# mschauer/ZigZagBoomerang.jl

Hardware: AMD Instinct MI355X
Metric: reflection events/sec, d=16384 local ZigZag (spdmp), ensemble of independent chains (higher is better)
Workload: dtype f64

## Files before the change

### include/pdmp_debug.h

```cpp
#ifndef PDMP_DEBUG_H
#define PDMP_DEBUG_H

#include <stddef.h>

#include "pdmp_mi355.h"

#ifdef __cplusplus
extern "C" {
#endif

#define PDMP_DEBUG_KERNEL_AUTO 0
#define PDMP_DEBUG_KERNEL_SEQ 1
#define PDMP_DEBUG_KERNEL_SPEC4 2
#define PDMP_DEBUG_KERNEL_SPEC8 3
#define PDMP_DEBUG_KERNEL_EXACTP 4
pdmp_status pdmp_debug_set_kernel(pdmp_ensemble* ens, int kernel);
pdmp_status pdmp_debug_set_spec_g2(pdmp_ensemble* ens, int on);
pdmp_status pdmp_debug_set_phase_profile(pdmp_ensemble* ens, int on);
pdmp_status pdmp_debug_phase_profile(pdmp_ensemble* ens, double* out16, int* kind);
pdmp_status pdmp_debug_set_track_groups(pdmp_ensemble* ens, int which);
pdmp_status pdmp_debug_set_helper_wave(pdmp_ensemble* ens, int mode);
pdmp_status pdmp_debug_set_track_lines(pdmp_ensemble* ens, int mode);
pdmp_status pdmp_debug_buffer_addresses(pdmp_ensemble* ens, uint64_t* out8);
pdmp_status pdmp_debug_placement(pdmp_ensemble* ens, char* buf, size_t nbuf);
pdmp_status pdmp_debug_set_placement(pdmp_ensemble* ens, int tune, int place, const char* rec, const char* kp, const char* ev);
pdmp_status pdmp_debug_move_buffer(pdmp_ensemble* ens, int which);
pdmp_status pdmp_debug_set_helper_steering(pdmp_ensemble* ens, double gain, int target, double ahead);
pdmp_status pdmp_debug_set_launch_count_limit(pdmp_ensemble* ens, uint32_t n);
pdmp_status pdmp_debug_set_consumer_overlap(pdmp_ensemble* ens, int mode);
pdmp_status pdmp_debug_host_drain_probe(pdmp_ensemble* ens, int64_t bytes, double* gbps);
pdmp_status pdmp_debug_last_kernel(pdmp_ensemble* ens, char* out, int64_t cap);
pdmp_status pdmp_debug_set_logistic_rows(pdmp_ensemble* ens, int row_width);
pdmp_status pdmp_debug_set_proposal_dump(pdmp_ensemble* ens, int64_t n);

pdmp_status pdmp_debug_math_probe(int device, uint64_t seed, int64_t n, double* out);

#define PDMP_MATH_U01 0
#define PDMP_MATH_LOG 1
#define PDMP_MATH_EXP 2
#define PDMP_MATH_SINCOS 3
#define PDMP_MATH_SINCOS2PI 4
#define PDMP_MATH_RANDN 5
#define PDMP_MATH_RANDN2 6
#define PDMP_MATH_RANDINT 7
// ... 41 lines not shown
```

### zigzagboomerang.jl_amd/_lib.py

```python
import ctypes as C
import os

import numpy as np

from . import build as _build

PDMP_OK = 0
ABI_VERSION = 3
ERR_NAMES = {0: "PDMP_OK", 1: "PDMP_ERR_INVALID", 2: "PDMP_ERR_NO_DEVICE", 3: "PDMP_ERR_HIP",
             4: "PDMP_ERR_UNSUPPORTED", 5: "PDMP_ERR_NOMEM"}

PDMP_ERR_INVALID, PDMP_ERR_NO_DEVICE, PDMP_ERR_HIP, PDMP_ERR_UNSUPPORTED, PDMP_ERR_NOMEM = 1, 2, 3, 4, 5
SAMPLER_ZIGZAG_LOCAL, SAMPLER_ZIGZAG_ALL, SAMPLER_BPS, SAMPLER_STICKY_ZIGZAG = 0, 1, 2, 3
CHAIN_OK, CHAIN_BOUND_VIOLATED, CHAIN_STALLED, CHAIN_TRACE_FULL, CHAIN_PAUSED = 0, 1, 2, 3, 4


def needs_rerun(status):
    st = np.asarray(status)
    return bool(np.any((st == CHAIN_TRACE_FULL) | (st == CHAIN_PAUSED)))
RUN_REFERENCE_TAIL, RUN_STOP_BEFORE = 0, 1

EVENT_DTYPE = np.dtype([("t", "<f8"), ("i", "<i8"), ("x", "<f8"), ("theta", "<f8")])
COUNTERS_DTYPE = np.dtype([("t_last", "<f8"), ("num", "<u8"), ("nacc", "<u8"), ("nrefresh", "<u8"),
                           ("ntrace", "<u8"), ("nevents", "<u8"), ("ndraw_main", "<u8"),
                           ("ndraw_global", "<u8"), ("status", "<u4"), ("reserved", "<u4")])
assert EVENT_DTYPE.itemsize == 32 and COUNTERS_DTYPE.itemsize == 72

EXPORTED_SYMBOLS = [
    "pdmp_last_error", "pdmp_abi_version", "pdmp_device_count", "pdmp_ensemble_create",
    "pdmp_ensemble_destroy", "pdmp_ensemble_set_flow_zigzag", "pdmp_ensemble_set_target_gaussian_csc",
    "pdmp_ensemble_set_state", "pdmp_ensemble_set_state_synthetic", "pdmp_ensemble_run", "pdmp_ensemble_run_partitioned", "pdmp_ensemble_sync",
    "pdmp_ensemble_last_run_ms", "pdmp_ensemble_counters", "pdmp_ensemble_totals", "pdmp_ensemble_trace_copy",
    "pdmp_ensemble_trace_reset", "pdmp_ensemble_final_state", "pdmp_ensemble_batch_means",
    "pdmp_ensemble_trace_dev", "pdmp_ensemble_counters_dev", 
    "pdmp_ensemble_set_flow_bps", "pdmp_ensemble_set_state_bps", "pdmp_ensemble_bps_trace_copy",
    "pdmp_ensemble_bps_final_state", "pdmp_ensemble_set_sticky", "pdmp_ensemble_set_adaptscale", "pdmp_ensemble_final_sigma", "pdmp_ensemble_set_flow_boomerang", "pdmp_ensemble_set_local_bound", "pdmp_ensemble_set_target_logistic", "pdmp_ensemble_set_flow_factboomerang",
    "pdmp_ensemble_set_mass_cholesky", "pdmp_ensemble_set_bps_options", "pdmp_ensemble_set_bps_moments", "pdmp_ensemble_bps_moments",
    "pdmp_ensemble_set_bps_sticky", "pdmp_ensemble_bps_trace_free_copy", "pdmp_ensemble_bps_final_sticky",
    "pdmp_ensemble_ess_begin", "pdmp_ensemble_ess_batch", "pdmp_ensemble_ess_end", "pdmp_ensemble_set_gradient_tracking",
    "pdmp_ensemble_path_integrals", "pdmp_ensemble_set_path_integrals", "pdmp_ensemble_set_neighbourhood", "pdmp_ensemble_info",
    "pdmp_ensemble_consume_begin", "pdmp_ensemble_consume", "pdmp_ensemble_consume_async", "pdmp_ensemble_last_consume_ms", "pdmp_ensemble_consume_mean", "pdmp_ensemble_consume_inclusion", "pdmp_ensemble_consume_discretized", "pdmp_ensemble_consume_cummean", "pdmp_ensemble_consume_cummean_copy", "pdmp_ensemble_subtrace_copy", "pdmp_1d_run",
    "pdmp_comm_unique_id", "pdmp_comm_init", "pdmp_comm_destroy", "pdmp_comm_info", "pdmp_comm_barrier", "pdmp_comm_allreduce",
    "pdmp_ensemble_gather_traces", "pdmp_ensemble_reduce_moments", "pdmp_comm_gathered_copy",
    "pdmp_ensemble_gather_bps_traces", "pdmp_comm_gathered_bps_copy", "pdmp_ensemble_bps_trace_dev",
]
DEBUG_SYMBOLS = ["pdmp_debug_set_kernel", "pdmp_debug_set_spec_g2", "pdmp_debug_set_phase_profile", "pdmp_debug_phase_profile",
                 "pdmp_debug_set_proposal_dump", "pdmp_debug_set_track_groups", "pdmp_debug_set_helper_wave", "pdmp_debug_set_track_lines", "pdmp_debug_buffer_addresses", "pdmp_debug_placement", "pdmp_debug_set_placement", "pdmp_debug_move_buffer", "pdmp_debug_set_helper_steering", "pdmp_debug_set_launch_count_limit", "pdmp_debug_host_drain_probe", "pdmp_debug_set_consumer_overlap", "pdmp_debug_last_kernel", "pdmp_debug_set_logistic_rows", "pdmp_debug_math_probe", "pdmp_debug_math_eval", "pdmp_debug_write_probe", "pdmp_debug_sector_probe",
                 "pdmp_debug_sticky_eval"]
DEBUG_KERNELS = {"auto": 0, "seq": 1, "spec4": 2, "spec8": 3, "exactp": 4}


class PdmpConfig(C.Structure):
    _fields_ = [("struct_size", C.c_uint32), ("device", C.c_int32), ("sampler", C.c_int32), ("adapt", C.c_int32),
                ("factor", C.c_double), ("nchains", C.c_int64), ("d", C.c_int64), ("trace_capacity", C.c_int64)]


class PdmpError(RuntimeError):
    def __init__(self, code, msg):
        super().__init__(f"{ERR_NAMES.get(code, code)}: {msg}")
        self.code = code


_lib = None
_loaded_path = None


def loaded_path():
    return _loaded_path


# ... 82 lines not shown
    L.pdmp_ensemble_set_flow_bps.argtypes = [vp, vp, vp, vp, vp, f64, f64]
    L.pdmp_ensemble_set_flow_boomerang.argtypes = [vp, vp, vp, vp, vp, vp, f64, f64]
    L.pdmp_ensemble_set_state_bps.argtypes = [vp, f64, vp, vp, f64, vp]
    L.pdmp_ensemble_ess_begin.argtypes = [vp, f64]
    L.pdmp_ensemble_ess_batch.argtypes = [vp, f64]
    L.pdmp_ensemble_ess_end.argtypes = [vp, vp, vp, vp, vp, C.POINTER(i64), C.POINTER(f64), C.POINTER(f64)]
    L.pdmp_ensemble_set_mass_cholesky.argtypes = [vp, vp, vp, vp]
    L.pdmp_ensemble_set_bps_options.argtypes = [vp, C.c_int, C.c_int]
    L.pdmp_ensemble_set_bps_moments.argtypes = [vp, C.c_int]
    L.pdmp_ensemble_bps_moments.argtypes = [vp, f64, i64, i64, vp, vp]
    L.pdmp_ensemble_set_bps_sticky.argtypes = [vp, vp, C.c_int]
    L.pdmp_ensemble_bps_trace_free_copy.argtypes = [vp, i64, i64, i64, vp]
    L.pdmp_ensemble_bps_final_sticky.argtypes = [vp, i64, i64, vp, vp]
    L.pdmp_debug_sticky_eval.argtypes = [C.c_int, C.c_int, i64, vp, vp, vp, vp]
    L.pdmp_ensemble_bps_trace_copy.argtypes = [vp, i64, i64, i64, vp, vp, vp]
    L.pdmp_ensemble_bps_final_state.argtypes = [vp, i64, i64, vp, vp, vp, vp]
    L.pdmp_debug_set_kernel.argtypes = [vp, C.c_int]
    L.pdmp_debug_set_spec_g2.argtypes = [vp, C.c_int]
    L.pdmp_debug_set_phase_profile.argtypes = [vp, C.c_int]
    L.pdmp_debug_phase_profile.argtypes = [vp, vp, C.POINTER(C.c_int)]
    L.pdmp_debug_set_proposal_dump.argtypes = [vp, i64]
    L.pdmp_debug_set_track_groups.argtypes = [vp, C.c_int]
    L.pdmp_debug_set_helper_wave.argtypes = [vp, C.c_int]
    L.pdmp_debug_set_track_lines.argtypes = [vp, C.c_int]
    L.pdmp_debug_buffer_addresses.argtypes = [vp, C.POINTER(C.c_uint64)]
    L.pdmp_debug_move_buffer.argtypes = [vp, C.c_int]
    L.pdmp_debug_placement.argtypes = [vp, C.c_char_p, C.c_size_t]
    L.pdmp_debug_set_placement.argtypes = [vp, C.c_int, C.c_int, C.c_char_p, C.c_char_p, C.c_char_p]
    L.pdmp_debug_set_launch_count_limit.argtypes = [vp, C.c_uint32]
    L.pdmp_debug_set_helper_steering.argtypes = [vp, C.c_double, C.c_int, C.c_double]
    L.pdmp_debug_last_kernel.argtypes = [vp, C.c_char_p, i64]
    L.pdmp_debug_set_logistic_rows.argtypes = [vp, C.c_int]
    for name in EXPORTED_SYMBOLS + DEBUG_SYMBOLS:
        fn = getattr(L, name)
        if name not in ("pdmp_last_error", "pdmp_abi_version", "pdmp_device_count", "pdmp_ensemble_destroy", "pdmp_comm_destroy"):
            fn.restype = C.c_int
    _lib = L
    _loaded_path = path
    return L


class Config1d(C.Structure):
    _fields_ = [("struct_size", C.c_uint32), ("device", C.c_int32), ("flow", C.c_int32), ("adapt", C.c_int32), ("factor", C.c_double),
                ("nchains", C.c_int64), ("trace_capacity", C.c_int64), ("mu", C.c_double), ("sigma2", C.c_double), ("noise", C.c_double),
                ("b_sigma", C.c_double), ("b_mu", C.c_double), ("b_lambda", C.c_double)]

# ... 41 lines not shown
```

### zigzagboomerang.jl_amd/csrc/pdmp_capi.hip

```cpp
#include <hip/hip_runtime.h>

#include <chrono>

#include <algorithm>
#include <cmath>
#include <cstdarg>
#include <cstdio>
#include <cstdlib>
#include <cstring>
#include <string>
#include <unordered_map>
#include <vector>

#include "../../include/pdmp_detmath.h"
#include "../../include/pdmp_debug.h"
#include "pdmp_engine.hpp"

namespace {

thread_local std::string g_err;
thread_local std::string g_deferred_err;

pdmp_status fail(pdmp_status st, const char* fmt, ...) {
    char buf[512];
// ... 81 lines not shown
    DevBuf<uint64_t> d_blob;
    DevBuf<uint32_t> d_tix;
    size_t n_templates = 0;
    uint32_t common_tix = 0;

    DevBuf<uint32_t> d_colptr, d_rowval, d_sptr, d_sidx, d_qptr;
    DevBuf<uint8_t> d_pos, d_selfpos;
    DevBuf<double> d_bval, d_tval, d_gmu_b, d_gmu_t, d_c, d_c2, d_sigma;
    DevBuf<pdmp::CoordConst> d_cc;
    DevBuf<pdmp::ZzRec> d_rec;
    DevBuf<double> d_keys, d_c_chain, d_jprev, d_sum;
    int dbg_kernel = 0;
    int dbg_lg_rows = -1;
    int dbg_spec_g2 = 0;
    int dbg_phase = 0;
    double dbg_phase_out[16] = {0};
    int dbg_phase_valid = 0;
    int64_t dbg_dump = 0;
    int dbg_track_groups = 0;
    double dbg_hw_steer[3] = {0, 0, 0};
    uint32_t dbg_count_limit = 0;
    int dbg_cons_overlap = -1;
    int n_cu = 0;
    int dbg_helper_wave = -1;
    bool track_requested = false, track = false, track_two_sums = false;
    bool track_lg = false;
    DevBuf<double> d_trk;
    bool exactp = false;
    bool track_pairs = false;
    DevBuf<double> d_kp;
    bool track_lines = false, canon_stale = false;
    pdmp::PlaceConfig place_cfg;
    int place_tune = 1;
    std::string tune_log;
    int dbg_track_lines = -1;
    DevBuf<pdmp::TrLine> d_tl_lines;
    DevBuf<pdmp::TrCold> d_tl_cold;
    bool has_g8 = false, g8_same = false;
    int g8_gw = 8;
    DevBuf<uint64_t> d_g8_line;
    DevBuf<double> d_g8_member, d_g8_gamt;
    bool track_generic = false;
    DevBuf<double> d_gam8;
    DevBuf<uint16_t> d_nb16;
    const char* last_kernel = "";
    int32_t lattice_n = 0;
// ... 416 lines not shown
        return hipSuccess;
    };
    switch (which) {
        case 0: HIP_TRY(move_buf(e->d_rec)); break;
        case 1: HIP_TRY(move_buf(e->d_kp)); break;
        case 2: HIP_TRY(move_buf(e->d_ev)); break;
        case 3: HIP_TRY(move_buf(e->d_hdr)); break;
        case 4: HIP_TRY(move_buf(e->d_cc)); break;
        case 5: HIP_TRY(move_buf(e->d_keys)); break;
        case 6: HIP_TRY(move_buf(e->b_ev_x)); break;
        case 7: HIP_TRY(move_buf(e->b_ev_th)); break;
        case 8: HIP_TRY(move_buf(e->b_x)); break;
        case 9: HIP_TRY(move_buf(e->b_th)); break;
        case 10: HIP_TRY(move_buf(e->b_ev_t)); break;
        default: return fail(PDMP_ERR_INVALID, "move buffer: 0 records, 1 pairs, 2 trace, 3 headers, 4 constants, 5 keys; BPS: 6 / 7 event x / theta, 8 / 9 x / theta, 10 event t");
    }
    return PDMP_OK;
}
pdmp_status pdmp_debug_set_helper_wave(pdmp_ensemble* e, int mode) {
    if (!e || mode < -1 || mode > 1) return fail(PDMP_ERR_INVALID, "helper wave: -1 (by occupancy), 0 (never), 1 (always)");
    e->dbg_helper_wave = mode;
    return PDMP_OK;
}
pdmp_status pdmp_debug_set_consumer_overlap(pdmp_ensemble* e, int mode) {
    if (!e || mode < -1 || mode > 1) return fail(PDMP_ERR_INVALID, "consumer overlap: -1 (by width), 0 (between slices), 1 (beside the next slice)");
    e->dbg_cons_overlap = mode;
    return PDMP_OK;
}
pdmp_status pdmp_debug_set_launch_count_limit(pdmp_ensemble* e, uint32_t n) {
    if (!e) return fail(PDMP_ERR_INVALID, "null argument");
    e->dbg_count_limit = n;
    return PDMP_OK;
}
pdmp_status pdmp_debug_set_helper_steering(pdmp_ensemble* e, double gain, int target, double ahead) {
    if (!e || !(gain > 0.0 && gain <= 4096.0) || target < 1 || target > 64 || !(ahead >= 0.0))
        return fail(PDMP_ERR_INVALID, "helper steering: 0 < gain <= 4096 (<= 1 for the two-wave form), 1 <= target <= 64, ahead >= 0");
    e->dbg_hw_steer[0] = gain;
    e->dbg_hw_steer[1] = (double)target;
    e->dbg_hw_steer[2] = ahead;
    return PDMP_OK;
}
pdmp_status pdmp_debug_set_logistic_rows(pdmp_ensemble* e, int w) {
    if (!e || (w != -1 && w != 0 && w != 16 && w != 32)) return fail(PDMP_ERR_INVALID, "row width: -1 (default), 0 (one chain per wavefront), 16 or 32");
#ifndef PDMP_EXTRA_KERNELS
    if (w > 0) return fail(PDMP_ERR_UNSUPPORTED, "zz_logistic_rows_kernel is not part of this library: it lives in the parity build (build.py --variant parity, -DPDMP_EXTRA_KERNELS)");
#endif
// ... 911 lines not shown
    if (general_path(e)) return P;
    if (e->track || e->exactp) {
        P.lattice_n = e->lattice_n;
        P.lattice_magic = e->lattice_n ? (uint32_t)(((uint64_t)1 << 32) / (uint64_t)e->lattice_n + 1) : 0u;
    }
    if (!e->track) return P;
    P.track_two_sums = e->track_two_sums ? 1 : 0;
    if (!e->track_pairs) return P;
    P.typ_extra = e->typ_extra;
    P.hw_gain = e->dbg_hw_steer[0];
    P.hw_target = (uint32_t)e->dbg_hw_steer[1];
    P.hw_ahead = e->dbg_hw_steer[2];
    if (e->track_lines) {
        P.tl_lines = e->d_tl_lines.p;
        P.tl_cold = e->d_tl_cold.p;
        return P;
    }
    P.keys = e->d_kp.p;
    P.track_mean = e->track_mean;
    if (e->track_mean == 2) P.tb.gmu_t = nullptr;
    P.n_cu = e->n_cu;
    P.helper_wave = (e->dbg_helper_wave == 1 || (e->dbg_helper_wave == -1 && e->cfg.nchains <= (int64_t)HELPER_WAVE_MAX_CHAINS_PER_CU * (e->n_cu > 0 ? e->n_cu : 256))) ? 1 : 0;
    if (pdmp::zz_trackp_big(e->cfg.d)) P.helper_wave = 0;
    return P;
}

static pdmp::ZzGeneralParams general_params(const pdmp_ensemble* e) {
    pdmp::ZzGeneralParams Q{};
    Q.local_bound = e->local_bound ? 1 : 0;
    Q.masked = e->has_g1mask ? 1 : 0;
    Q.sticky = e->cfg.sampler == PDMP_SAMPLER_STICKY_ZIGZAG ? 1 : 0;
    Q.qtval = e->d_qtval.p;
    Q.renew_chain = e->local_bound ? e->d_thf.p : nullptr;
    Q.sig_chain = e->adaptscale ? e->d_sig_chain.p : nullptr;
    Q.adaptscale = e->adaptscale ? 1 : 0;
    Q.pos16 = e->d_pos16.p;
    Q.qbval = e->d_qbval.p;
    Q.member = reinterpret_cast<const uint4*>(e->d_member.p);
    Q.selfpos16 = e->d_selfpos16.p;
    Q.mmax_pad = (e->mmax_all + 63u) & ~63u;
    Q.target_kind = e->target_kind;
    Q.A_colptr = e->lg_Acp.p;
    Q.A_rowval = e->lg_Arv.p;
    Q.A_nzval = e->lg_Anz.p;
    Q.At_colptr = e->lg_Atcp.p;
    Q.At_rowval = e->lg_Atrv.p;
// ... 184 lines not shown

static pdmp::BpsRunParams bps_run_params(const pdmp_ensemble* e, double T, int flags);
static pdmp::BpsMomParams bps_moments_params(const pdmp_ensemble* e);
static pdmp::BpsStickyParams bps_sticky_params(const pdmp_ensemble* e);

pdmp_status pdmp_ensemble_run(pdmp_ensemble* e, double T, int flags, void* stream) {
    pdmp_status st = ensemble_run_impl(e, T, flags, stream);
    if (st == PDMP_OK && e->cfg.sampler != PDMP_SAMPLER_BPS) e->run_T = T;
    if (st == PDMP_OK && e->deferred_k >= 0) st = launch_deferred_consumer(e);
    return st;
}

static pdmp_status ensemble_run_impl(pdmp_ensemble* e, double T, int flags, void* stream) {
    if (!e) return fail(PDMP_ERR_INVALID, "null argument");
    if (!e->has_state) return fail(PDMP_ERR_INVALID, "set_state must be called before run");
    if (flags != PDMP_RUN_REFERENCE_TAIL && flags != PDMP_RUN_STOP_BEFORE) return fail(PDMP_ERR_INVALID, "bad flags");
    HIP_TRY(hipSetDevice(e->cfg.device));
    e->ran = true;
    hipStream_t s = stream ? (hipStream_t)stream : e->stream;
    const int64_t n = e->cfg.nchains;
    const bool bps = e->cfg.sampler == PDMP_SAMPLER_BPS;
    pdmp_status st;
    if (!bps) e->dbg_phase_valid = 0;
    if (!bps && general_path(e) && e->lg_nemax >= 1024 && !e->d_hot.p && (st = e->d_hot.alloc((size_t)n * (size_t)e->cfg.d * 4)) != PDMP_OK) return st;
    const pdmp::BpsRunParams B = bps_run_params(e, T, flags);
    pdmp::ZzRunParams P = run_params(e, T, flags);
    const pdmp::ZzGeneralParams Q = general_params(e);
    const pdmp::ZzLogisticTables LT = logistic_tables(e);
    KernelFamily fam;
    if ((st = select_family(e, P, Q, LT, &fam)) != PDMP_OK) return st;
    const FamilyInfo& F = FAMILY[fam];
    DevBuf<double> dbgbuf, phbuf;
    const int64_t dbg_cap = bps ? 0 : e->dbg_dump;
    if (dbg_cap > 0) {
        if ((st = dbgbuf.alloc((size_t)dbg_cap * 16)) != PDMP_OK) return st;
        HIP_TRY(hipMemsetAsync(dbgbuf.p, 0, (size_t)dbg_cap * 16 * sizeof(double), s));
        P.dbg = dbgbuf.p;
        P.dbg_cap = dbg_cap;
    }
    HIP_TRY(hipEventRecord(e->ev0, s));
    const bool profiled = e->dbg_phase != 0 && F.phase_kind != 0;
    if (profiled) {
        if ((st = phbuf.alloc(16)) != PDMP_OK) return st;
        HIP_TRY(hipMemsetAsync(phbuf.p, 0, 16 * sizeof(double), s));
        P.dbg = phbuf.p;
        P.dbg_cap = 0;
    }
    int rc = 0;
    switch (fam) {
    case FAM_BPS:
        if (e->bps_sticky) {
            e->last_kernel = "bps_sticky_run_kernel";
            rc = pdmp::launch_bps_sticky_run(B, bps_sticky_params(e), n, s);
        } else {
            e->last_kernel = "bps_run_kernel";
            rc = pdmp::launch_bps_run(B, n, e->bps_diag, s, bps_moments_params(e));
        }
        break;
    case FAM_GENERAL: e->last_kernel = "zz_general_run_kernel"; rc = pdmp::launch_zz_general_run(P, Q, n, s); break;
    case FAM_LOGISTIC_LDS: e->last_kernel = "zz_logistic_lds_kernel"; rc = pdmp::launch_zz_logistic_lds(P, Q, LT, e->keep_integrals, n, s); break;
    case FAM_TRACKL: e->last_kernel = "zz_local_trackl_kernel"; e->canon_stale = true; rc = pdmp::launch_zz_local_trackl(P, n, s); break;
    case FAM_TRACKP: rc = pdmp::launch_zz_local_trackp(P, n, s, &e->last_kernel); break;
    case FAM_TRACK_GROUPS: e->last_kernel = "zz_local_track_kernel"; rc = pdmp::launch_zz_local_track(P, n, s); break;
    case FAM_STICKY_SPEC: e->last_kernel = "zz_sticky_spec_kernel"; rc = pdmp::launch_zz_sticky_spec(P, n, s); break;
    case FAM_STICKY_RUN: e->last_kernel = "zz_sticky_run_kernel"; rc = pdmp::launch_zz_sticky_run(P, n, s); break;
    case FAM_SPEC: rc = pdmp::launch_zz_local_spec(P, n, s, &e->last_kernel); break;
    case FAM_ONE_EVENT: e->last_kernel = "zz_local_run_kernel"; rc = pdmp::launch_zz_local_run(P, n, s); break;
#ifdef PDMP_EXTRA_KERNELS
    case FAM_LOGISTIC_ROWS: e->last_kernel = "zz_logistic_rows_kernel"; rc = pdmp::launch_zz_logistic_rows(P, Q, LT, e->keep_integrals, logistic_rows_width(e), n, s); break;
    case FAM_EXACTP: e->last_kernel = "zz_local_exactp_kernel"; rc = pdmp::launch_zz_local_exactp(P, n, s); break;
#else
    case FAM_LOGISTIC_ROWS: case FAM_EXACTP: return fail(PDMP_ERR_UNSUPPORTED, "kernel family %d is not part of this library", (int)fam);
#endif
    }
    if (rc != 0 && F.hip_rc) return fail(PDMP_ERR_HIP, "%s launch failed: %s", F.launcher, hipGetErrorString((hipError_t)rc));
    if (rc != 0) return fail(PDMP_ERR_HIP, "%s launch failed (%d)", F.launcher, rc);
    HIP_TRY(hipEventRecord(e->ev1, s));
    e->timed = true;
    if (profiled) {
        HIP_TRY(device_sync(e));
        HIP_TRY(hipMemcpy(e->dbg_phase_out, phbuf.p, sizeof e->dbg_phase_out, hipMemcpyDeviceToHost));
        e->dbg_phase_valid = F.phase_kind;
    }
    if (dbg_cap > 0 && (fam == FAM_ONE_EVENT || fam == FAM_STICKY_RUN)) {
        HIP_TRY(device_sync(e));
        std::vector<double> hd((size_t)dbg_cap * 16);
        HIP_TRY(hipMemcpy(hd.data(), dbgbuf.p, hd.size() * sizeof(double), hipMemcpyDeviceToHost));
        for (int64_t r = 0; r < dbg_cap; ++r) {
            const double* D = hd.data() + r * 16;
            fprintf(stderr, "DBG %3lld tp=%.6f i=%g acc=%g k=%g m=%g self=%g l=%.6g lb=%.6g u=%.6f key=%.6f t=%.6f L=%.6f g=%.6g a_i=%.6g x0=%.6g cj=%.6g\n",
                    (long long)r, D[0], D[1], D[2], D[3], D[4], D[5], D[6], D[7], D[8], D[9], D[10], D[11], D[12], D[13], D[14], D[15]);
        }
    }
    return PDMP_OK;
}

pdmp_status pdmp_ensemble_sync(pdmp_ensemble* e) {
    if (!e) return fail(PDMP_ERR_INVALID, "null argument");
    HIP_TRY(hipSetDevice(e->cfg.device));
    HIP_TRY(device_sync(e));
    return PDMP_OK;
}

pdmp_status pdmp_ensemble_last_run_ms(pdmp_ensemble* e, float* ms) {
    if (!e || !ms) return fail(PDMP_ERR_INVALID, "null argument");
// ... 1226 lines not shown
```

### zigzagboomerang.jl_amd/csrc/pdmp_engine.hpp

```cpp
#pragma once
#include <cstdint>
#include <string>
#include <vector>

#include "../../include/pdmp_mi355.h"
#ifdef PDMP_EXTRA_KERNELS
#include "../../include/pdmp_debug.h"
#endif

namespace pdmp {

struct alignas(64) ZzRec {
    double x;
    double th;
    double t;
    double I;
    double t_old;
    double a, b;
    uint64_t acc;
};
static_assert(sizeof(ZzRec) == 64, "record must be one 64-byte sector");

struct alignas(128) TrRec {
    double x, th, tx, I;
// ... 98 lines not shown
    uint32_t blob_w, blob_w_pad, blob_sw, blob_pw, blob_kmax;
    uint32_t common_tix;
    int64_t d;
    int64_t dk;
    int64_t trace_cap;
    uint32_t nblk;
    uint32_t nblk_pad;
    double T;
    double factor;
    double lambda_ref;
    int32_t flags;
    int32_t adapt;
    int32_t has_refresh;
    int32_t move_all;
    int32_t force_spec4;
    int32_t track_two_sums;
    int32_t track_mean;
    uint32_t count_limit;
    uint32_t typ_extra;
    double hw_gain, hw_ahead;
    uint32_t hw_target;
    int32_t n_cu;
    int32_t helper_wave;
    void* tl_lines;
    void* tl_cold;
    int32_t lattice_n;
    uint32_t lattice_magic;
    const uint64_t* __restrict__ g8_line;
    const double* __restrict__ g8_member;
    const double* __restrict__ g8_gamt;
    int32_t g8_gw;
    const double* __restrict__ kappa;
    double* thf;
    int32_t reversible, strong_upperbounds;
};

struct ZzInitParams {
    ZzTables tb;
    ZzRec* rec;
    double* keys;
    DevChain* hdr;
    double* c_chain;
    const double* x0;
    const double* th0;
    const uint64_t* seeds;
    uint64_t seed0;
// ... 256 lines not shown
```

### zigzagboomerang.jl_amd/csrc/pdmp_trackp.hip

```cpp
#include <hip/hip_runtime.h>

#include <cstdint>

#include "../../include/pdmp_detmath.h"
#include "pdmp_device.hpp"
#include "pdmp_engine.hpp"

namespace pdmp {

namespace {

__device__ __forceinline__ uint32_t w_grp8_min_u32(uint32_t v) {
    uint32_t o = (uint32_t)__builtin_amdgcn_mov_dpp((int)v, 0xB1, 0xf, 0xf, true);
    v = (o < v) ? o : v;
    o = (uint32_t)__builtin_amdgcn_mov_dpp((int)v, 0x4E, 0xf, 0xf, true);
    v = (o < v) ? o : v;
    o = (uint32_t)__builtin_amdgcn_mov_dpp((int)v, 0x141, 0xf, 0xf, true);
    return (o < v) ? o : v;
}
__device__ __forceinline__ uint32_t p_enc(double key, double tb, uint32_t pos) {
    double dlt = key - tb;
    dlt = (dlt > 0.0) ? dlt : 0.0;
    const uint32_t b = __float_as_uint((float)dlt);
    return (((b >= 8u) ? b - 8u : 0u) & ~7u) | pos;
// ... 221 lines not shown
        uint32_t e = P_INFBITS;
        if (b < nblk) {
            const double2* p = kp + (size_t)b * 8;
            double mk = p[0].x;
            uint32_t mi = 0;
#pragma unroll
            for (int q = 1; q < 8; ++q) {
                const double v = p[q].x;
                if (v < mk) {
                    mk = v;
                    mi = q;
                }
            }
            e = (mk < PDMP_INF) ? p_enc(mk, tb, mi) : P_INFBITS;
        }
        lbf[b] = e;
    }
    PDMP_LDS_ORDER();

    uint64_t ph[10] = {0, 0, 0, 0, 0, 0, 0, 0, 0, 0};
    uint64_t ph_t0 = PROF ? (uint64_t)__builtin_readcyclecounter() : 0;
    uint64_t ph_rounds = 0, ph_guess = 0;
    uint64_t ph_iters = 0, ph_raw = 0, ph_zone = 0, ph_eval = 0;
#ifdef PDMP_PHASE_MARKS
#define WMARK(k) asm volatile("; WPHASE " #k)
#else
#define WMARK(k)
#endif
#define WPHASE(k)                                                         \
    do {                                                                  \
        WMARK(k);                                                         \
        if (PROF) {                                                       \
            const uint64_t now_ = (uint64_t)__builtin_readcyclecounter(); \
            ph[k] += now_ - ph_t0;                                        \
            ph_t0 = now_;                                                 \
        }                                                                 \
    } while (0)

    PrioTurn prio;
    bool need_rebase = false;
    uint32_t idle = 0;
    bool running = stop_before || (t_event < T);
    while (running) {
        prio.step();
        if (dnacc >= trace_room) {
            status = PDMP_CHAIN_TRACE_FULL;
// ... 41 lines not shown
        bool stalled = false, finished = false;
        double dt_used = 0.0;
        uint32_t Cc = 0;
        double tau = 0.0, mql_sel = 0.0;
        bool tau_clipped = false;
        {
            uint32_t kk[32];
            auto loadc = [&](int c) {
#pragma unroll
                for (int j = 0; j < 8; ++j) {
                    const uint4 v = reinterpret_cast<const uint4*>(lbf)[512 * c + lane + 64 * j];
                    kk[4 * j + 0] = v.x;
                    kk[4 * j + 1] = v.y;
                    kk[4 * j + 2] = v.z;
                    kk[4 * j + 3] = v.w;
                }
            };
            auto lanemin = [&]() -> uint32_t {
                uint32_t m_ = kk[0];
#pragma unroll
                for (int j = 1; j < 32; ++j) m_ = (kk[j] < m_) ? kk[j] : m_;
                return m_;
            };
            uint32_t mloc = 0xffffffffu;
#pragma unroll
            for (int c = 0; c < NCH; ++c) {
                loadc(c);
                const uint32_t m_ = lanemin();
                mloc = (m_ < mloc) ? m_ : mloc;
            }
            uint32_t mqb = wave_min_u32_dpp(mloc);
            double mql = p_dec(mqb, tb);
            if (mqb < P_INFBITS && (need_rebase || mql - tb > 0.25)) {
                mloc = 0xffffffffu;
#pragma unroll
                for (int c = 0; c < NCH; ++c) {
                    if (NCH > 1) loadc(c);
#pragma unroll
                    for (int j = 0; j < 32; ++j)
                        kk[j] = (kk[j] >= P_INFBITS) ? P_INFBITS : p_enc(p_dec(kk[j], tb), mql, kk[j] & 7u);
#pragma unroll
                    for (int j = 0; j < 8; ++j)
                        reinterpret_cast<uint4*>(lbf)[512 * c + lane + 64 * j] = make_uint4(kk[4 * j + 0], kk[4 * j + 1], kk[4 * j + 2], kk[4 * j + 3]);
                    const uint32_t m_ = lanemin();
                    mloc = (m_ < mloc) ? m_ : mloc;
                }
                tb = mql;
                need_rebase = false;
                mqb = wave_min_u32_dpp(mloc);
                mql = p_dec(mqb, tb);
                PDMP_LDS_ORDER();
            }
            if (mqb >= P_INFBITS) {
                stalled = true;
            } else if (stop_before && !(mql < T)) {
                finished = true;
            } else {
                double dt_sel = seldt;
                uint32_t cm[NCH], ncl = 0, incl = 0;
                for (int tries = 0;; ++tries) {
                    tau = mql + dt_sel;
                    tau_clipped = false;
                    if (stop_before && !(tau < T)) {
                        tau = pdmp_below(T);
                        tau_clipped = true;
                    }
                    if (tries >= 64) tau = mql;
                    const uint32_t thr0 = p_thr(tau, tb), thr = (thr0 < P_INFBITS) ? thr0 : P_INFBITS - 1u;
                    ncl = 0;
#pragma unroll
                    for (int c = 0; c < NCH; ++c) {
                        if (NCH > 1) loadc(c);
                        uint32_t m_ = 0;
#pragma unroll
                        for (int j = 31; j >= 0; --j) m_ = m_ + m_ + ((kk[j] <= thr) ? 1u : 0u);
                        cm[c] = m_;
                        ncl += (uint32_t)__builtin_popcount(m_);
                    }
                    incl = scan_add_u32(ncl);
                    Cc = (uint32_t)__builtin_amdgcn_readlane((int)incl, 63);
                    if (Cc <= (uint32_t)W_CMAX || tries >= 64) break;
                    dt_sel *= HW ? (double)(W_CMAX - 6) / (double)Cc : 0.5;
                }
                {
                    uint32_t ix = incl - ncl;
#pragma unroll
                    for (int c = 0; c < NCH; ++c) {
                        uint32_t m_ = cm[c];
                        while (__ballot(m_ != 0u) != 0) {
                            if (m_ != 0u) {
                                const uint32_t j = (uint32_t)(__ffs((int)m_) - 1);
                                if (ix < 64u) TB[ix] = (uint16_t)(2048u * (uint32_t)c + 4u * ((uint32_t)lane + 64u * (j >> 2)) + (j & 3u));
                                ix += 1;
                                m_ &= m_ - 1u;
                            }
                        }
                    }
                }
// ... 414 lines not shown
                if (mem) gam = (gl == 0) ? ria->gam0 : (gl == 1) ? ria->gam1 : (gl == 2) ? ria->gam2 : (gl == 3) ? ria->gam3 : ria->gam4;
            } else {
                if (mem) gam = P.tb.gam8[(size_t)ia * 8 + (size_t)gl];
            }
            const double th_ia = ria->th;
            double xa = ria->x, txa = ria->tx, Ia = ria->I;
            const uint64_t acc_ia = ria->acc;
            const double thj0 = rj->th, gj0 = rj->g, gdj0 = rj->gd, tgj = rj->tg;
            double gmu_j = 0.0;
            if (tmean) gmu_j = rj->tacc;
            double2 cjm2 = *reinterpret_cast<const double2*>(&rj->c);
            asm volatile("" : "+v"(cjm2.x), "+v"(cjm2.y));
            const double resta_b = bperm_f64(rest, ea);
            const uint32_t rarga_b = (uint32_t)__builtin_amdgcn_ds_bpermute((int)(ea << 2), (int)rarg);
            const bool selfl = mem && jm == ia;
            const bool adapted = selfl && ((vb_adapt >> ea) & 1ull) != 0ull;
            if (adapted) {
                cjm2.x = cjm2.x * P.factor;
                cjm2.y = cjm2.x / 100;
            }
            const double thj = selfl ? -th_ia : thj0;
            const double gj = gj0 + gdj0 * (tpa - tgj);
            const double gdj = gdj0 + gam * (-2.0 * th_ia);
            double a2l, b2l, key2l;
            {
                const bool mine = gact || !first;
                const uint32_t dix = mine ? (offa + 1u + (uint32_t)gl) : (off + 1u);
                const double Lg = drawlog(dnm + ((dix < W_WIN - 1u) ? dix : W_WIN - 1u));
                const double cc = mine ? cjm2.x : c_i, cc100 = mine ? cjm2.y : c_i2.y;
                const double gg0 = mine ? gj : g_now, tt = mine ? thj : th, gdd = mine ? gdj : gd_i;
                const double gg = tmean ? gg0 - (mine ? gmu_j : gmu_i) : gg0;
                a2l = cc + gg * tt;
                b2l = cc100 + tt * gdd;
                key2l = (mine ? tpa : tp) + poisson_time_L(a2l, b2l, Lg);
            }
            const double keyj = mem ? key2l : PDMP_INF;
            if (first) {
                if (__ballot(ev && !acc && gact) != 0) {
                    const double Le = drawlog(dnm + ((off + 1u < W_WIN - 1u) ? off + 1u : W_WIN - 1u));
                    const double a2e = c_i + (tmean ? g_now - gmu_i : g_now) * th;
                    const double b2e = c_i2.y + th * gd_i;
                    const double k2e = tp + poisson_time_L(a2e, b2e, Le);
                    if (gact) key2l = k2e;
                }
                key2 = key2l;
            }
            if (selfl) {
                const double dtx = tpa - txa;
                const double xn = xa + th_ia * dtx;
                Ia = Ia + dtx * ((xa + xn) * 0.5);
                xa = xn;
                txa = tpa;
            }
            const double kin = (mem && (jm >> 3) == blka) ? keyj : PDMP_INF;
            const double kinmin = grp8_min_f64(kin);
            const uint32_t wkey = (gact && kin == kinmin) ? (((uint32_t)gl << 3) | (jm & 7u)) : 0xffu;
            const uint32_t jwin = w_grp8_min_u32(wkey);
            const bool restwins = resta_b <= kinmin;
            const double rowmin_a = restwins ? resta_b : kinmin;
            const uint32_t cand_a = restwins ? (rarga_b & 7u) : (jwin & 7u);
            const double keymin = grp8_min_f64(keyj);
            if (gact && gl == 0) EX[ea] = min_f64(rowmin_a, keymin);
            asm volatile("" ::"v"(xa), "v"(txa), "v"(Ia), "v"(acc_ia));
            o.gact = gact;
            o.mem = mem;
            o.selfl = selfl;
            o.adapted = adapted;
            o.c_new = cjm2.x;
// ... 114 lines not shown
        }
        if (vsel >= 0) {
            const double tpv = readlane_f64(tp, vsel);
            const uint32_t iv = (uint32_t)__builtin_amdgcn_readlane((int)i, vsel);
            if (lane == 0) kp[iv].y = tpv;
            dnum += 1;
            vnacc = 1;
            dnm += 1;
            t_last = tpv;
            status = PDMP_CHAIN_BOUND_VIOLATED;
        }
        if (status != PDMP_CHAIN_OK) break;
        PDMP_LDS_ORDER();
    }

    if (PROF && P.dbg && chain == 0 && lane == 0) {
        for (int q = 0; q < 10; ++q) P.dbg[q] = (double)ph[q];
        P.dbg[10] = (double)ph_iters;
        P.dbg[11] = (double)ph_raw;
        P.dbg[12] = (double)ph_zone;
        P.dbg[13] = (double)ph_eval;
        P.dbg[14] = (double)ph_rounds;
        P.dbg[15] = (double)ph_guess;
    }
#undef WPHASE
    if (HW && lane == 0) ctl->exitf = 1u;
    if (lane == 0) {
        hdr->c.t_last = t_last;
        hdr->t_event = t_event;
        hdr->c.num += dnum;
        hdr->c.nacc += dnacc + vnacc;
        hdr->c.ntrace = ntrace0 + dnacc;
        hdr->c.nevents += dnacc;
        hdr->c.ndraw_main = nm0 + dnm;
        hdr->c.status = status;
    }
}

template <bool PROF, bool LAT>
__global__ __launch_bounds__(64) __attribute__((amdgpu_waves_per_eu(4, 4))) void zz_local_trackp_kernel(ZzRunParams P) {
    trackp_body<PROF, LAT, false, false>(P);
}
template <bool PROF>
__global__ __launch_bounds__(64) __attribute__((amdgpu_waves_per_eu(1, 2))) void zz_local_trackp_big_kernel(ZzRunParams P) {
    trackp_body<PROF, true, false, true>(P);
}
// ... 126 lines not shown
```

### zigzagboomerang.jl_amd/engine.py

```python
import ctypes as C
import os

import numpy as np

from . import _lib
from .flows import BouncyParticle, FactBoomerang, GaussianTarget, LogisticTarget, ZigZag


def _i64(a):
    return np.ascontiguousarray(a, dtype=np.int64)


def _f64(a):
    return np.ascontiguousarray(a, dtype=np.float64)


def _ptr(a):
    return None if a is None else a.ctypes.data


class Ensemble:

    def __init__(self, nchains, d, *, sampler=_lib.SAMPLER_ZIGZAG_LOCAL, adapt=False, factor=1.8, device=0,
                 trace_capacity=0):
        self._L = _lib.load()
        self.nchains, self.d = int(nchains), int(d)
        self.trace_capacity = int(trace_capacity)
        self.adapt = bool(adapt)
        self.device = int(device)
        self._bps_mom = 0
        cfg = _lib.PdmpConfig(C.sizeof(_lib.PdmpConfig), int(device), int(sampler), int(bool(adapt)), float(factor),
                              self.nchains, self.d, self.trace_capacity)
        h = C.c_void_p()
        _lib.check(self._L.pdmp_ensemble_create(C.byref(cfg), C.byref(h)))
        self._h = h
        k = os.environ.get("PDMP_KERNEL")
        if k:
            self.debug_set_kernel(k)
        if os.environ.get("PDMP_TRACK_GROUPS"):
            _lib.check(self._L.pdmp_debug_set_track_groups(self._h, int(os.environ["PDMP_TRACK_GROUPS"])))
        if os.environ.get("PDMP_HELPER_WAVE"):
            self.debug_set_helper_wave(int(os.environ["PDMP_HELPER_WAVE"]))
        if os.environ.get("PDMP_TRACK_LINES"):
            self.debug_set_track_lines(int(os.environ["PDMP_TRACK_LINES"]))
        if any(os.environ.get(v) for v in ("PDMP_PLACE_TUNE", "PDMP_PLACE", "PDMP_PLACE_rec", "PDMP_PLACE_kp", "PDMP_PLACE_ev")):
            pat = [os.environ.get("PDMP_PLACE_" + a, "").encode() or None for a in ("rec", "kp", "ev")]
            self.debug_set_placement(int(os.environ.get("PDMP_PLACE_TUNE", "-1")), int(os.environ.get("PDMP_PLACE", "1" if any(pat) else "0")), *pat)
        if os.environ.get("PDMP_LAUNCH_COUNT_LIMIT"):
            _lib.check(self._L.pdmp_debug_set_launch_count_limit(self._h, int(os.environ["PDMP_LAUNCH_COUNT_LIMIT"])))
        if os.environ.get("PDMP_HELPER_STEER"):
            g_, k_, a_ = os.environ["PDMP_HELPER_STEER"].split(",")
            _lib.check(self._L.pdmp_debug_set_helper_steering(self._h, float(g_), int(k_), float(a_)))
        if os.environ.get("PDMP_LG_ROWS"):
            _lib.check(self._L.pdmp_debug_set_logistic_rows(self._h, int(os.environ["PDMP_LG_ROWS"])))
        if os.environ.get("PDMP_SPEC_G2"):
            _lib.check(self._L.pdmp_debug_set_spec_g2(self._h, 1))

    def debug_set_kernel(self, name):
        _lib.check(self._L.pdmp_debug_set_kernel(self._h, _lib.DEBUG_KERNELS[name]))

    def debug_set_helper_wave(self, mode):
        _lib.check(self._L.pdmp_debug_set_helper_wave(self._h, int(mode)))

    def debug_set_track_lines(self, mode):
        _lib.check(self._L.pdmp_debug_set_track_lines(self._h, int(mode)))

    def debug_buffer_addresses(self):
        import ctypes as C
        out = (C.c_uint64 * 8)()
        _lib.check(self._L.pdmp_debug_buffer_addresses(self._h, out))
        return dict(zip(("trk", "kp", "ev", "hdr", "rec", "keys", "cc", "blob"), [int(v) for v in out]))

    def debug_set_placement(self, tune=-1, place=0, rec=None, kp=None, ev=None):
        _lib.check(self._L.pdmp_debug_set_placement(self._h, int(tune), int(place), rec, kp, ev))

    def debug_placement(self):
        import ctypes
        buf = ctypes.create_string_buffer(1024)
        _lib.check(self._L.pdmp_debug_placement(self._h, buf, 1024))
        return buf.value.decode()

    def debug_move_buffer(self, which):
        _lib.check(self._L.pdmp_debug_move_buffer(self._h, int(which)))

    def kernel_name(self):
# ... 355 lines not shown
```

Measured before the change: 1.392 billion.

## Serve rejected-lane re-bound proposals from idle lanes instead of a second pass

In the tracked-proposal ZigZag kernel, when an event is rejected on a lane that is also updating a neighbour, the second Poisson-time proposal is now computed by an idle lane. The operands are exchanged via LDS lane tables and ds_bpermute, replacing a wave-wide second drawlog/poisson_time pass. The rebase loop is restructured to skip a redundant min recomputation, and the threshold bitmask uses alignbit. This adds LDS traffic and permutes, and falls back to the two-pass path when there are too few idle lanes; debug counters and a mode switch are added.

```diff
diff --git a/include/pdmp_debug.h b/include/pdmp_debug.h
--- a/include/pdmp_debug.h
+++ b/include/pdmp_debug.h
@@ -20,6 +20,8 @@
 pdmp_status pdmp_debug_phase_profile(pdmp_ensemble* ens, double* out16, int* kind);
 pdmp_status pdmp_debug_set_track_groups(pdmp_ensemble* ens, int which);
 pdmp_status pdmp_debug_set_helper_wave(pdmp_ensemble* ens, int mode);
+pdmp_status pdmp_debug_set_rebound_passes(pdmp_ensemble* ens, int mode);
+pdmp_status pdmp_debug_rebound_stats(pdmp_ensemble* ens, uint64_t* out3);
 pdmp_status pdmp_debug_set_track_lines(pdmp_ensemble* ens, int mode);
 pdmp_status pdmp_debug_buffer_addresses(pdmp_ensemble* ens, uint64_t* out8);
 pdmp_status pdmp_debug_placement(pdmp_ensemble* ens, char* buf, size_t nbuf);
diff --git a/zigzagboomerang.jl_amd/_lib.py b/zigzagboomerang.jl_amd/_lib.py
--- a/zigzagboomerang.jl_amd/_lib.py
+++ b/zigzagboomerang.jl_amd/_lib.py
@@ -45,7 +45,7 @@
     "pdmp_ensemble_gather_bps_traces", "pdmp_comm_gathered_bps_copy", "pdmp_ensemble_bps_trace_dev",
 ]
 DEBUG_SYMBOLS = ["pdmp_debug_set_kernel", "pdmp_debug_set_spec_g2", "pdmp_debug_set_phase_profile", "pdmp_debug_phase_profile",
-                 "pdmp_debug_set_proposal_dump", "pdmp_debug_set_track_groups", "pdmp_debug_set_helper_wave", "pdmp_debug_set_track_lines", "pdmp_debug_buffer_addresses", "pdmp_debug_placement", "pdmp_debug_set_placement", "pdmp_debug_move_buffer", "pdmp_debug_set_helper_steering", "pdmp_debug_set_launch_count_limit", "pdmp_debug_host_drain_probe", "pdmp_debug_set_consumer_overlap", "pdmp_debug_last_kernel", "pdmp_debug_set_logistic_rows", "pdmp_debug_math_probe", "pdmp_debug_math_eval", "pdmp_debug_write_probe", "pdmp_debug_sector_probe",
+                 "pdmp_debug_set_proposal_dump", "pdmp_debug_set_track_groups", "pdmp_debug_set_helper_wave", "pdmp_debug_set_rebound_passes", "pdmp_debug_rebound_stats", "pdmp_debug_set_track_lines", "pdmp_debug_buffer_addresses", "pdmp_debug_placement", "pdmp_debug_set_placement", "pdmp_debug_move_buffer", "pdmp_debug_set_helper_steering", "pdmp_debug_set_launch_count_limit", "pdmp_debug_host_drain_probe", "pdmp_debug_set_consumer_overlap", "pdmp_debug_last_kernel", "pdmp_debug_set_logistic_rows", "pdmp_debug_math_probe", "pdmp_debug_math_eval", "pdmp_debug_write_probe", "pdmp_debug_sector_probe",
                  "pdmp_debug_sticky_eval"]
 DEBUG_KERNELS = {"auto": 0, "seq": 1, "spec4": 2, "spec8": 3, "exactp": 4}
 
@@ -174,6 +174,8 @@
     L.pdmp_debug_set_proposal_dump.argtypes = [vp, i64]
     L.pdmp_debug_set_track_groups.argtypes = [vp, C.c_int]
     L.pdmp_debug_set_helper_wave.argtypes = [vp, C.c_int]
+    L.pdmp_debug_set_rebound_passes.argtypes = [vp, C.c_int]
+    L.pdmp_debug_rebound_stats.argtypes = [vp, vp]
     L.pdmp_debug_set_track_lines.argtypes = [vp, C.c_int]
     L.pdmp_debug_buffer_addresses.argtypes = [vp, C.POINTER(C.c_uint64)]
     L.pdmp_debug_move_buffer.argtypes = [vp, C.c_int]
diff --git a/zigzagboomerang.jl_amd/csrc/pdmp_capi.hip b/zigzagboomerang.jl_amd/csrc/pdmp_capi.hip
--- a/zigzagboomerang.jl_amd/csrc/pdmp_capi.hip
+++ b/zigzagboomerang.jl_amd/csrc/pdmp_capi.hip
@@ -127,6 +127,9 @@
     uint32_t dbg_count_limit = 0;
     int dbg_cons_overlap = -1;
     int n_cu = 0;
+    int dbg_rebound_passes = -1;
+    uint64_t dbg_rebound_stats[3] = {0, 0, 0};
+    int dbg_rebound_valid = 0;
     int dbg_helper_wave = -1;
     bool track_requested = false, track = false, track_two_sums = false;
     bool track_lg = false;
@@ -589,6 +592,17 @@
     e->dbg_helper_wave = mode;
     return PDMP_OK;
 }
+pdmp_status pdmp_debug_set_rebound_passes(pdmp_ensemble* e, int mode) {
+    if (!e || (mode != -1 && mode != 2)) return fail(PDMP_ERR_INVALID, "rebound passes: -1 (displaced proposals in idle lanes where they suffice), 2 (always a second pass)");
+    e->dbg_rebound_passes = mode;
+    return PDMP_OK;
+}
+pdmp_status pdmp_debug_rebound_stats(pdmp_ensemble* e, uint64_t* out3) {
+    if (!e || !out3) return fail(PDMP_ERR_INVALID, "null argument");
+    if (!e->dbg_rebound_valid) return fail(PDMP_ERR_INVALID, "no re-bound statistics recorded by the last run");
+    memcpy(out3, e->dbg_rebound_stats, sizeof e->dbg_rebound_stats);
+    return PDMP_OK;
+}
 pdmp_status pdmp_debug_set_consumer_overlap(pdmp_ensemble* e, int mode) {
     if (!e || mode < -1 || mode > 1) return fail(PDMP_ERR_INVALID, "consumer overlap: -1 (by width), 0 (between slices), 1 (beside the next slice)");
     e->dbg_cons_overlap = mode;
@@ -1546,6 +1560,7 @@
     P.n_cu = e->n_cu;
     P.helper_wave = (e->dbg_helper_wave == 1 || (e->dbg_helper_wave == -1 && e->cfg.nchains <= (int64_t)HELPER_WAVE_MAX_CHAINS_PER_CU * (e->n_cu > 0 ? e->n_cu : 256))) ? 1 : 0;
     if (pdmp::zz_trackp_big(e->cfg.d)) P.helper_wave = 0;
+    P.rebound_passes = e->dbg_rebound_passes;
     return P;
 }
 
@@ -1776,6 +1791,7 @@
     const bool bps = e->cfg.sampler == PDMP_SAMPLER_BPS;
     pdmp_status st;
     if (!bps) e->dbg_phase_valid = 0;
+    if (!bps) e->dbg_rebound_valid = 0;
     if (!bps && general_path(e) && e->lg_nemax >= 1024 && !e->d_hot.p && (st = e->d_hot.alloc((size_t)n * (size_t)e->cfg.d * 4)) != PDMP_OK) return st;
     const pdmp::BpsRunParams B = bps_run_params(e, T, flags);
     pdmp::ZzRunParams P = run_params(e, T, flags);
@@ -1795,8 +1811,8 @@
     HIP_TRY(hipEventRecord(e->ev0, s));
     const bool profiled = e->dbg_phase != 0 && F.phase_kind != 0;
     if (profiled) {
-        if ((st = phbuf.alloc(16)) != PDMP_OK) return st;
-        HIP_TRY(hipMemsetAsync(phbuf.p, 0, 16 * sizeof(double), s));
+        if ((st = phbuf.alloc(16 + 3)) != PDMP_OK) return st;
+        HIP_TRY(hipMemsetAsync(phbuf.p, 0, (16 + 3) * sizeof(double), s));
         P.dbg = phbuf.p;
         P.dbg_cap = 0;
     }
@@ -1835,6 +1851,12 @@
         HIP_TRY(device_sync(e));
         HIP_TRY(hipMemcpy(e->dbg_phase_out, phbuf.p, sizeof e->dbg_phase_out, hipMemcpyDeviceToHost));
         e->dbg_phase_valid = F.phase_kind;
+        if (fam == FAM_TRACKP) {
+            double rb[3];
+            HIP_TRY(hipMemcpy(rb, phbuf.p + 16, sizeof rb, hipMemcpyDeviceToHost));
+            for (int q = 0; q < 3; ++q) e->dbg_rebound_stats[q] = (uint64_t)rb[q];
+            e->dbg_rebound_valid = 1;
+        }
     }
     if (dbg_cap > 0 && (fam == FAM_ONE_EVENT || fam == FAM_STICKY_RUN)) {
         HIP_TRY(device_sync(e));
diff --git a/zigzagboomerang.jl_amd/csrc/pdmp_engine.hpp b/zigzagboomerang.jl_amd/csrc/pdmp_engine.hpp
--- a/zigzagboomerang.jl_amd/csrc/pdmp_engine.hpp
+++ b/zigzagboomerang.jl_amd/csrc/pdmp_engine.hpp
@@ -144,6 +144,7 @@
     uint32_t hw_target;
     int32_t n_cu;
     int32_t helper_wave;
+    int32_t rebound_passes;
     void* tl_lines;
     void* tl_cold;
     int32_t lattice_n;
diff --git a/zigzagboomerang.jl_amd/csrc/pdmp_trackp.hip b/zigzagboomerang.jl_amd/csrc/pdmp_trackp.hip
--- a/zigzagboomerang.jl_amd/csrc/pdmp_trackp.hip
+++ b/zigzagboomerang.jl_amd/csrc/pdmp_trackp.hip
@@ -267,6 +267,7 @@
     uint64_t ph_t0 = PROF ? (uint64_t)__builtin_readcyclecounter() : 0;
     uint64_t ph_rounds = 0, ph_guess = 0;
     uint64_t ph_iters = 0, ph_raw = 0, ph_zone = 0, ph_eval = 0;
+    uint64_t ph_rb_iters = 0, ph_rb_disp = 0, ph_rb_fall = 0;
 #ifdef PDMP_PHASE_MARKS
 #define WMARK(k) asm volatile("; WPHASE " #k)
 #else
@@ -354,33 +355,35 @@
                 for (int j = 1; j < 32; ++j) m_ = (kk[j] < m_) ? kk[j] : m_;
                 return m_;
             };
-            uint32_t mloc = 0xffffffffu;
-#pragma unroll
-            for (int c = 0; c < NCH; ++c) {
-                loadc(c);
-                const uint32_t m_ = lanemin();
-                mloc = (m_ < mloc) ? m_ : mloc;
-            }
-            uint32_t mqb = wave_min_u32_dpp(mloc);
-            double mql = p_dec(mqb, tb);
-            if (mqb < P_INFBITS && (need_rebase || mql - tb > 0.25)) {
-                mloc = 0xffffffffu;
+            uint32_t mqb;
+            double mql;
+            for (bool rebased = false;; rebased = true) {
+                uint32_t mloc = 0xffffffffu;
+#pragma unroll
+                for (int c = 0; c < NCH; ++c) {
+                    loadc(c);
+                    const uint32_t m_ = lanemin();
+                    mloc = (m_ < mloc) ? m_ : mloc;
+                }
+                mqb = wave_min_u32_dpp(mloc);
+                mql = p_dec(mqb, tb);
+                if (rebased || !(mqb < P_INFBITS && (need_rebase || mql - tb > 0.25))) break;
 #pragma unroll
                 for (int c = 0; c < NCH; ++c) {
                     if (NCH > 1) loadc(c);
 #pragma unroll
-                    for (int j = 0; j < 32; ++j)
-                        kk[j] = (kk[j] >= P_INFBITS) ? P_INFBITS : p_enc(p_dec(kk[j], tb), mql, kk[j] & 7u);
-#pragma unroll
-                    for (int j = 0; j < 8; ++j)
-                        reinterpret_cast<uint4*>(lbf)[512 * c + lane + 64 * j] = make_uint4(kk[4 * j + 0], kk[4 * j + 1], kk[4 * j + 2], kk[4 * j + 3]);
-                    const uint32_t m_ = lanemin();
-                    mloc = (m_ < mloc) ? m_ : mloc;
+                    for (int j = 0; j < 8; ++j) {
+                        uint32_t nk[4];
+#pragma unroll
+                        for (int q = 0; q < 4; ++q) {
+                            const uint32_t k_ = kk[4 * j + q];
+                            nk[q] = (k_ >= P_INFBITS) ? P_INFBITS : p_enc(p_dec(k_, tb), mql, k_ & 7u);
+                        }
+                        reinterpret_cast<uint4*>(lbf)[512 * c + lane + 64 * j] = make_uint4(nk[0], nk[1], nk[2], nk[3]);
+                    }
                 }
                 tb = mql;
                 need_rebase = false;
-                mqb = wave_min_u32_dpp(mloc);
-                mql = p_dec(mqb, tb);
                 PDMP_LDS_ORDER();
             }
             if (mqb >= P_INFBITS) {
@@ -405,7 +408,8 @@
                         if (NCH > 1) loadc(c);
                         uint32_t m_ = 0;
 #pragma unroll
-                        for (int j = 31; j >= 0; --j) m_ = m_ + m_ + ((kk[j] <= thr) ? 1u : 0u);
+                        for (int j = 31; j >= 0; --j) m_ = __builtin_amdgcn_alignbit(m_, thr - kk[j], 31u);
+                        m_ = ~m_;
                         cm[c] = m_;
                         ncl += (uint32_t)__builtin_popcount(m_);
                     }
@@ -866,28 +870,60 @@
             const double thj = selfl ? -th_ia : thj0;
             const double gj = gj0 + gdj0 * (tpa - tgj);
             const double gdj = gdj0 + gam * (-2.0 * th_ia);
-            double a2l, b2l, key2l;
+            const bool two_pass = P.rebound_passes == 2;
+            const bool mine = (two_pass ? gact : mem) || !first;
+            const bool rej = ev && !acc;
+            const uint64_t dispb = first ? __ballot(rej && mine) : 0ull, idleb = first ? __ballot(!rej && !mine) : 0ull;
+            const uint32_t ndisp = (uint32_t)__popcll(dispb);
+            const bool serve = !two_pass && ndisp != 0u && ndisp <= (uint32_t)__popcll(idleb);
+            double key2l, ptl, keyj;
+            uint32_t srv = (uint32_t)lane;
             {
-                const bool mine = gact || !first;
-                const uint32_t dix = mine ? (offa + 1u + (uint32_t)gl) : (off + 1u);
+                const double a2e = c_i + (tmean ? g_now - gmu_i : g_now) * th;
+                const double b2e = c_i2.y + th * gd_i;
+                const double a2m = cjm2.x + (tmean ? gj - gmu_j : gj) * thj;
+                const double b2m = cjm2.y + thj * gdj;
+                double a2l = mine ? a2m : a2e, b2l = mine ? b2m : b2e;
+                uint32_t dix = mine ? (offa + 1u + (uint32_t)gl) : (off + 1u);
+                if (serve) {
+                    const uint32_t rd = __builtin_amdgcn_mbcnt_hi((uint32_t)(dispb >> 32), __builtin_amdgcn_mbcnt_lo((uint32_t)dispb, 0u));
+                    const uint32_t ri = __builtin_amdgcn_mbcnt_hi((uint32_t)(idleb >> 32), __builtin_amdgcn_mbcnt_lo((uint32_t)idleb, 0u));
+                    const bool disp = rej && mine, serving = !rej && !mine && ri < ndisp;
+                    PDMP_LDS_ORDER();
+                    if (disp) TB[rd] = (uint16_t)lane;
+                    if (serving) TB[32u + ri] = (uint16_t)lane;
+                    PDMP_LDS_ORDER();
+                    const uint32_t src = serving ? (uint32_t)TB[ri] : (uint32_t)lane;
+                    if (disp) srv = (uint32_t)TB[32u + rd];
+                    PDMP_LDS_ORDER();
+                    double pa = bperm_f64(a2e, src), pb = bperm_f64(b2e, src);
+                    uint32_t po = (uint32_t)__builtin_amdgcn_ds_bpermute((int)(src << 2), (int)(off + 1u));
+                    asm volatile("" : "+v"(pa), "+v"(pb), "+v"(po), "+v"(srv));
+                    a2l = serving ? pa : a2l;
+                    b2l = serving ? pb : b2l;
+                    dix = serving ? po : dix;
+                }
                 const double Lg = drawlog(dnm + ((dix < W_WIN - 1u) ? dix : W_WIN - 1u));
-                const double cc = mine ? cjm2.x : c_i, cc100 = mine ? cjm2.y : c_i2.y;
-                const double gg0 = mine ? gj : g_now, tt = mine ? thj : th, gdd = mine ? gdj : gd_i;
-                const double gg = tmean ? gg0 - (mine ? gmu_j : gmu_i) : gg0;
-                a2l = cc + gg * tt;
-                b2l = cc100 + tt * gdd;
-                key2l = (mine ? tpa : tp) + poisson_time_L(a2l, b2l, Lg);
-            }
-            const double keyj = mem ? key2l : PDMP_INF;
+                ptl = poisson_time_L(a2l, b2l, Lg);
+                key2l = (mine ? tpa : tp) + ptl;
+                keyj = mem ? key2l : PDMP_INF;
+                if (!serve && ndisp != 0u) {
+                    const double Le = drawlog(dnm + ((off + 1u < W_WIN - 1u) ? off + 1u : W_WIN - 1u));
+                    const double k2e = tp + poisson_time_L(a2e, b2e, Le);
+                    if (mine) key2l = k2e;
+                }
+            }
             if (first) {
-                if (__ballot(ev && !acc && gact) != 0) {
-                    const double Le = drawlog(dnm + ((off + 1u < W_WIN - 1u) ? off + 1u : W_WIN - 1u));
-                    const double a2e = c_i + (tmean ? g_now - gmu_i : g_now) * th;
-                    const double b2e = c_i2.y + th * gd_i;
-                    const double k2e = tp + poisson_time_L(a2e, b2e, Le);
-                    if (gact) key2l = k2e;
+                if (serve) {
+                    const double pts = bperm_f64(ptl, srv);
+                    if (rej && mine) key2l = tp + pts;
                 }
                 key2 = key2l;
+                if (PROF) {
+                    ph_rb_iters += 1;
+                    ph_rb_disp += (ndisp != 0u) ? 1u : 0u;
+                    ph_rb_fall += (ndisp != 0u && !serve) ? 1u : 0u;
+                }
             }
             if (selfl) {
                 const double dtx = tpa - txa;
@@ -1048,6 +1084,9 @@
         P.dbg[13] = (double)ph_eval;
         P.dbg[14] = (double)ph_rounds;
         P.dbg[15] = (double)ph_guess;
+        P.dbg[16] = (double)ph_rb_iters;
+        P.dbg[17] = (double)ph_rb_disp;
+        P.dbg[18] = (double)ph_rb_fall;
     }
 #undef WPHASE
     if (HW && lane == 0) ctl->exitf = 1u;
diff --git a/zigzagboomerang.jl_amd/engine.py b/zigzagboomerang.jl_amd/engine.py
--- a/zigzagboomerang.jl_amd/engine.py
+++ b/zigzagboomerang.jl_amd/engine.py
@@ -41,6 +41,8 @@
             _lib.check(self._L.pdmp_debug_set_track_groups(self._h, int(os.environ["PDMP_TRACK_GROUPS"])))
         if os.environ.get("PDMP_HELPER_WAVE"):
             self.debug_set_helper_wave(int(os.environ["PDMP_HELPER_WAVE"]))
+        if os.environ.get("PDMP_REBOUND_PASSES"):
+            self.debug_set_rebound_passes(int(os.environ["PDMP_REBOUND_PASSES"]))
         if os.environ.get("PDMP_TRACK_LINES"):
             self.debug_set_track_lines(int(os.environ["PDMP_TRACK_LINES"]))
         if any(os.environ.get(v) for v in ("PDMP_PLACE_TUNE", "PDMP_PLACE", "PDMP_PLACE_rec", "PDMP_PLACE_kp", "PDMP_PLACE_ev")):
@@ -61,6 +63,14 @@
 
     def debug_set_helper_wave(self, mode):
         _lib.check(self._L.pdmp_debug_set_helper_wave(self._h, int(mode)))
+
+    def debug_set_rebound_passes(self, mode):
+        _lib.check(self._L.pdmp_debug_set_rebound_passes(self._h, int(mode)))
+
+    def debug_rebound_stats(self):
+        out = np.zeros(3, dtype=np.uint64)
+        _lib.check(self._L.pdmp_debug_rebound_stats(self._h, _ptr(out)))
+        return tuple(int(v) for v in out)
 
     def debug_set_track_lines(self, mode):
         _lib.check(self._L.pdmp_debug_set_track_lines(self._h, int(mode)))
```

New measurement: 1.391 billion. About the same (-0.1%).
